# tensorflow/recommenders

Hardware: AMD Instinct MI355X
Metric: queries/sec brute-force top-100 (higher is better)
Workload: dtype f32; 1 GPU; BruteForce top-100, 1M-item x dim-64 corpus, batch 8192 (BASELINE.json configs[1]); corpus_rows_total=1000000, corpus_rows_per_gpu=1000000, dim=64, batch=8192, k=100, parallelism=single GPU

## Files before the change

recommenders_amd/csrc/topk_select16.hip:

```cpp
#include "common.h"

namespace tfrs {

constexpr int kSel16Waves = 4;
constexpr int kSlots = 16;
#ifndef TFRS_LIST16_ABLATE
#define TFRS_LIST16_ABLATE 0
#endif
#if TFRS_LIST16_ABLATE
#ifndef TFRS_ALLOW_ABLATION
#error "TFRS_LIST16_ABLATE != 0 is a measurement build with wrong results: add -DTFRS_ALLOW_ABLATION to confirm"
#endif
extern "C" int tfrs_ablation_build_list16(void) { return TFRS_LIST16_ABLATE; }
#endif
constexpr int kRadixBits = 24;

__device__ __forceinline__ uint32_t sel16_mbcnt(uint64_t mask) {
  return __builtin_amdgcn_mbcnt_hi((uint32_t)(mask >> 32),
                                   __builtin_amdgcn_mbcnt_lo((uint32_t)mask, 0u));
}
__device__ __forceinline__ void sel16_lds_sync() {
  __builtin_amdgcn_fence(__ATOMIC_ACQ_REL, "wavefront");
  __builtin_amdgcn_wave_barrier();
}

__device__ __forceinline__ uint32_t radix_kth(const uint32_t (&key)[kSlots], int k, int nslots = kSlots) {
  uint32_t kmax = 0u, kmin = 0xFFFFFFFFu;
  int n = 0;
#pragma unroll
  for (int s = 0; s < kSlots; ++s)
    if (s < nslots) {
      kmax = max(kmax, key[s]);
      kmin = min(kmin, key[s] != 0u ? key[s] : 0xFFFFFFFFu);
      n += (int)__popcll(__ballot(key[s] != 0u));
    }
  if (n < k) return 0u;
#pragma unroll
  for (int off = 32; off > 0; off >>= 1) {
    kmax = max(kmax, (uint32_t)__shfl_xor((int)kmax, off));
    kmin = min(kmin, (uint32_t)__shfl_xor((int)kmin, off));
  }
  kmax = __builtin_amdgcn_readfirstlane(kmax);
  kmin = __builtin_amdgcn_readfirstlane(kmin);
  constexpr uint32_t kLowBits = (1u << (32 - kRadixBits)) - 1u;
  const uint32_t diff = kmax ^ kmin;
  if ((diff & ~kLowBits) == 0u) return kmax & ~kLowBits;
  const int top = 31 - __builtin_clz(diff);
  uint32_t prefix = top == 31 ? 0u : (kmax & ~((2u << top) - 1u));
#pragma unroll 1
  for (int bit = top; bit >= 32 - kRadixBits; --bit) {
    const uint32_t test = prefix | (1u << bit);
    const uint32_t himask = ~((1u << bit) - 1u);
    int cnt = 0;
#pragma unroll
    for (int s = 0; s < kSlots; ++s)
      if (s < nslots) cnt += (int)__popcll(__ballot((key[s] & himask) == test));
    if (cnt >= k) prefix = test; else k -= cnt;
  }
  return prefix;
}

__global__ void __launch_bounds__(kSel16Waves * 64) bin_threshold_kernel(
    const float *__restrict__ binmax, int64_t ld, int n_bins, int group, int64_t nq, int k,
    const float *__restrict__ qk, const float *__restrict__ norm_max, float *__restrict__ lower,
    float *__restrict__ raw) {
  const int lane = threadIdx.x & 63;
  const int64_t row = (int64_t)blockIdx.x * kSel16Waves + (threadIdx.x >> 6);
  if (row >= nq) return;
  const float *src = binmax + row * ld;
  uint32_t key[kSlots];
  if (group == 1) {
    float v[kSlots];
#pragma unroll
    for (int s = 0; s < kSlots; ++s) {
      const int b = s * 64 + lane;
      v[s] = src[b < n_bins ? b : n_bins - 1];
    }
#pragma unroll
    for (int s = 0; s < kSlots; ++s) key[s] = (s * 64 + lane < n_bins) ? f32_orderable(v[s]) : 0u;
  } else
#pragma unroll
  for (int s = 0; s < kSlots; ++s) {
    const int b0 = (s * 64 + lane) * group;
    float m = -__builtin_inff();
    if (group % 4 == 0) {
      for (int g = 0; g < group; g += 4) {
        if (b0 + g + 3 < n_bins) {
          const float4 v = *reinterpret_cast<const float4 *>(src + b0 + g);
          m = fmaxf(fmaxf(m, fmaxf(v.x, v.y)), fmaxf(v.z, v.w));
        } else {
          for (int e = 0; e < 4; ++e)
            if (b0 + g + e < n_bins) m = fmaxf(m, src[b0 + g + e]);
        }
      }
    } else {
      for (int g = 0; g < group; ++g)
        if (b0 + g < n_bins) m = fmaxf(m, src[b0 + g]);
    }
    key[s] = (b0 < n_bins) ? f32_orderable(m) : 0u;
  }
  const int nslots = min(kSlots, (n_bins + group * 64 - 1) / (group * 64));
  const uint32_t kth = radix_kth(key, k, nslots);
  if (lane == 0) {
    const float eps = qk[row] * norm_max[0] + kF16Tiny;
    const bool have = kth > f32_orderable(-__builtin_inff());
    lower[row] = have ? f32_from_orderable(kth) - eps : -__builtin_inff();
    raw[row] = have ? f32_from_orderable(kth) : -__builtin_inff();
  }
}

int launch_bin_threshold(const float *binmax, int64_t ld, int n_bins, int64_t nq, int k,
                         const float *qk, const float *norm_max, float *lower, float *raw,
                         hipStream_t stream) {
  if (nq <= 0) return TFRS_OK;
  int group = 1;
  if (n_bins > 64 * kSlots) group = ((n_bins + 64 * kSlots - 1) / (64 * kSlots) + 3) / 4 * 4;
  hipLaunchKernelGGL(bin_threshold_kernel, dim3((unsigned)((nq + kSel16Waves - 1) / kSel16Waves)),
                     dim3(kSel16Waves * 64), 0, stream, binmax, ld, n_bins, group, nq, k, qk,
                     norm_max, lower, raw);
  TFRS_LAUNCH_CHECK();
  return TFRS_OK;
}

__device__ __forceinline__ float packed_score16(const char *packed, int64_t row, int dp,
                                                const float *qs) {
  const float4 *ev = reinterpret_cast<const float4 *>(packed + row * (int64_t)row_bytes(dp));
  const float4 *od = ev + dp / 8;
  const float4 *q4 = reinterpret_cast<const float4 *>(qs);
  float acc = 0.0f;
#pragma unroll 4
  for (int m = 0; m < dp / 8; ++m) {
    const float4 e = ev[m], o = od[m];
    const float4 qa = q4[2 * m], qb = q4[2 * m + 1];
    acc = __builtin_fmaf(e.x, qa.x, acc);
    acc = __builtin_fmaf(o.x, qa.y, acc);
    acc = __builtin_fmaf(e.y, qa.z, acc);
    acc = __builtin_fmaf(o.y, qa.w, acc);
    acc = __builtin_fmaf(e.z, qb.x, acc);
    acc = __builtin_fmaf(o.z, qb.y, acc);
    acc = __builtin_fmaf(e.w, qb.z, acc);
    acc = __builtin_fmaf(o.w, qb.w, acc);
  }
  return acc;
}

template <int P>
__device__ __forceinline__ void sort_desc16(uint64_t *x, int lane) {
#pragma unroll 1
  for (int size = 2; size <= P; size <<= 1) {
#pragma unroll 1
    for (int stride = size >> 1; stride > 0; stride >>= 1) {
      for (int t = lane; t < P / 2; t += 64) {
        const int i = 2 * t - (t & (stride - 1));
        const int jx = i + stride;
        const bool desc = ((i & size) == 0);
        const uint64_t va = x[i], vb = x[jx];
        if ((va < vb) == desc) {
          x[i] = vb;
          x[jx] = va;
        }
      }
      sel16_lds_sync();
    }
  }
}

struct List16Args {
  int64_t nq;
  int k;
  const float *q;
  int d;
  const char *packed;
  const uint2 *buf;
  const uint32_t *cnt;
  uint32_t cap_l;
  int nseg;
  const float *qk;
  const float *norm_max;
  float *out_scores;
  int32_t *out_idx;
  uint32_t *redo;
  int64_t idx_base;
  const uint32_t *ovf_cnt;
  const uint2 *ovf_buf;
  uint32_t ovf_cap;
  const int32_t *rowmap;
  const float *verify_raw;
  uint32_t *redo_reason;
  const RawTable *raw;
};

template <int KP>
__global__ void __launch_bounds__(kSel16Waves * 64) list_topk16_kernel(const List16Args a) {
  extern __shared__ __attribute__((aligned(16))) char smem[];
  const int lane = threadIdx.x & 63;
  const int wave = __builtin_amdgcn_readfirstlane(threadIdx.x >> 6);
  const int64_t row = (int64_t)blockIdx.x * kSel16Waves + wave;
  if (row >= a.nq) return;
  constexpr int kCap = 64 * kSlots;
  uint2 *ent = reinterpret_cast<uint2 *>(smem) + (size_t)wave * kCap;
  uint64_t *ex = reinterpret_cast<uint64_t *>(ent);
  float *qs = reinterpret_cast<float *>(smem + (size_t)kSel16Waves * kCap * sizeof(uint2)) +
              (size_t)wave * TFRS_MAX_DIM;
  const int K = a.k;
  const int dp = padded_dim(a.d);
  for (int i = lane; i < dp; i += 64) qs[i] = (i < a.d) ? a.q[row * a.d + i] : 0.0f;

  const uint2 *qbuf = a.buf + (row * (int64_t)a.cap_l) * a.nseg;
  int total = 0;
  bool bad = false;
  auto push = [&](bool p, uint2 v) __attribute__((always_inline)) {
    const uint64_t mask = __ballot(p);
    const int pos = total + (int)sel16_mbcnt(mask);
    if (p && pos < kCap) ent[pos] = v;
    total += (int)__popcll(mask);
  };
  constexpr int kCntBatch = 16;
  if (a.nseg <= 64) {
    const int lseg = lane < a.nseg ? lane : a.nseg - 1;
    const uint32_t ecap = a.cap_l - 1u;
    uint32_t c = a.cnt[row * a.nseg + lseg];
    if (lane >= a.nseg) c = 0u;
    if (a.ovf_cnt) {
      bad = c > a.cap_l + kOvfPerSeg;
      c = min(c, a.cap_l);
    } else {
      bad = c > a.cap_l;
    }
    if (__ballot(bad) == 0ull) {
      for (uint32_t e0 = 0; __ballot(e0 < c) != 0ull; e0 += 8) {
        uint2 w[8];
#pragma unroll
        for (int x = 0; x < 8; ++x) w[x] = qbuf[(int64_t)min(e0 + x, ecap) * a.nseg + lseg];
#pragma unroll
        for (int x = 0; x < 8; ++x) push(e0 + x < c, w[x]);
      }
    }
  } else
  for (int sb0 = 0; sb0 < a.nseg && !bad; sb0 += 64 * kCntBatch) {
    uint32_t cnts[kCntBatch];
#pragma unroll
    for (int b = 0; b < kCntBatch; ++b) {
      const int sg = sb0 + b * 64 + lane;
      cnts[b] = a.cnt[row * a.nseg + (sg < a.nseg ? sg : a.nseg - 1)];
    }
#pragma unroll
    for (int b = 0; b < kCntBatch; ++b)
      if (sb0 + b * 64 + lane >= a.nseg) cnts[b] = 0u;
#pragma unroll
    for (int b = 0; b < kCntBatch; ++b) {
      if (a.ovf_cnt) {
        bad = bad || (cnts[b] > a.cap_l + kOvfPerSeg);
        cnts[b] = min(cnts[b], a.cap_l);
      } else {
        bad = bad || (cnts[b] > a.cap_l);
      }
    }
    if (__ballot(bad) != 0ull) {
      bad = true;
      break;
    }
    uint2 v[kCntBatch][2];
#pragma unroll
    for (int b = 0; b < kCntBatch; ++b)
#pragma unroll
      for (int e = 0; e < 2; ++e) {
        const int sg = sb0 + b * 64 + lane;
        v[b][e] = qbuf[(int64_t)min((uint32_t)e, a.cap_l - 1u) * a.nseg + (sg < a.nseg ? sg : a.nseg - 1)];
      }
#pragma unroll
    for (int b = 0; b < kCntBatch; ++b) {
      if (sb0 + b * 64 >= a.nseg) break;
#pragma unroll
      for (int e = 0; e < 2; ++e) push((uint32_t)e < cnts[b], v[b][e]);
      for (uint32_t e0 = 2; __ballot(e0 < cnts[b]) != 0ull; e0 += 4) {
        uint2 w[4];
#pragma unroll
        for (int x = 0; x < 4; ++x) {
          const int sg = sb0 + b * 64 + lane;
          w[x] = qbuf[(int64_t)min(e0 + x, a.cap_l - 1u) * a.nseg + (sg < a.nseg ? sg : a.nseg - 1)];
        }
#pragma unroll
        for (int x = 0; x < 4; ++x) push(e0 + x < cnts[b], w[x]);
      }
    }
  }
  if (a.ovf_cnt && __ballot(bad) == 0ull) {
    const uint32_t novf = a.ovf_cnt[row];
    if (novf > a.ovf_cap) bad = true;
    else
      for (uint32_t e0 = 0; e0 < novf; e0 += 64) {
        const bool p = e0 + lane < novf;
        push(p, p ? a.ovf_buf[row * (int64_t)a.ovf_cap + e0 + lane] : make_uint2(0u, 0u));
      }
  }
  const bool any_bad = __ballot(bad) != 0ull;
  if (lane == 0 && a.redo_reason && total > 3 * kCap / 4 && !any_bad)
    atomicMax(&a.redo_reason[3], (uint32_t)total);
  if (any_bad || total > kCap) {
    if (lane == 0) a.redo[1 + atomicAdd(a.redo, 1u)] = (uint32_t)row;
    if (lane == 0 && a.redo_reason) atomicAdd(&a.redo_reason[0], 1u);
    return;
  }
  sel16_lds_sync();
  if (TFRS_LIST16_ABLATE & 4) { if (lane == 0) a.out_idx[row * K] = total; return; }

  uint32_t key[kSlots], rowid[kSlots];
#pragma unroll
  for (int s = 0; s < kSlots; ++s) {
    const int e = s * 64 + lane;
    key[s] = 0u;
    rowid[s] = 0u;
    if (e < total) {
      const uint2 v = ent[e];
      key[s] = f32_orderable(__uint_as_float(v.x));
      rowid[s] = v.y;
    }
  }
  const float eps = a.qk[row] * a.norm_max[0] + kF16Tiny;
  const uint32_t kth = radix_kth(key, K, (total + 63) / 64);
  if (a.verify_raw && (kth == 0u || kth < f32_orderable(a.verify_raw[row]))) {
    if (lane == 0) a.redo[1 + atomicAdd(a.redo, 1u)] = (uint32_t)row;
    if (lane == 0 && a.redo_reason) atomicAdd(&a.redo_reason[1], 1u);
    return;
  }
  uint32_t lo_key = 0u;
  if (kth != 0u && eps < __builtin_inff()) lo_key = f32_orderable(f32_from_orderable(kth) - 2.0f * eps);
  sel16_lds_sync();

  uint32_t *keep = reinterpret_cast<uint32_t *>(ent);
  int m = 0;
#pragma unroll
  for (int s = 0; s < kSlots; ++s) {
    const bool kp = key[s] != 0u && key[s] >= lo_key;
    const uint64_t mask = __ballot(kp);
    const int pos = m + (int)sel16_mbcnt(mask);
    if (kp && pos < kCap) keep[pos] = rowid[s];
    m += (int)__popcll(mask);
  }
  if (m > KP) {
    if (lane == 0 && a.redo_reason) atomicAdd(&a.redo_reason[2], 1u);
    sel16_lds_sync();
    uint32_t kall[kSlots];
#pragma unroll
    for (int u = 0; u < kSlots; ++u) kall[u] = (u * 64 + lane < m) ? keep[u * 64 + lane] : 0u;
    sel16_lds_sync();
#pragma unroll 1
    for (int u = 0; u < kSlots; ++u) {
      uint64_t kk = 0ull;
      if (u * 64 + lane < m)
        kk = make_key(a.raw ? raw_score(a.raw, (int64_t)kall[u], a.d, qs) : packed_score16(a.packed, (int64_t)kall[u], dp, qs),
                      (int32_t)((a.rowmap ? (int64_t)a.rowmap[kall[u]] : (int64_t)kall[u]) + a.idx_base));
      ex[u * 64 + lane] = kk;
    }
    sel16_lds_sync();
    sort_desc16<kCap>(ex, lane);
    for (int i = lane; i < K; i += 64) {
      const uint64_t kk = ex[i];
      a.out_scores[row * K + i] = kk ? key_score(kk) : -__builtin_inff();
      a.out_idx[row * K + i] = kk ? key_index(kk) : -1;
    }
    return;
  }
  sel16_lds_sync();
  uint32_t kid[KP / 64];
#pragma unroll
  for (int u = 0; u < KP / 64; ++u) kid[u] = (u * 64 + lane < m) ? keep[u * 64 + lane] : 0u;
  sel16_lds_sync();
#pragma unroll
  for (int u = 0; u < KP / 64; ++u) {
    if (u * 64 < m) {
      uint64_t kk = 0ull;
      if (u * 64 + lane < m)
        kk = make_key((TFRS_LIST16_ABLATE & 1) ? (float)kid[u] * 1e-9f :
                      a.raw ? raw_score(a.raw, (int64_t)kid[u], a.d, qs) : packed_score16(a.packed, (int64_t)kid[u], dp, qs),
                      (int32_t)((a.rowmap ? (int64_t)a.rowmap[kid[u]] : (int64_t)kid[u]) + a.idx_base));
      ex[u * 64 + lane] = kk;
    }
  }
  for (int i = m + lane; i < KP; i += 64) ex[i] = 0ull;
  sel16_lds_sync();
  if (!(TFRS_LIST16_ABLATE & 2)) {
    if (KP > 128 && m <= 128) sort_desc16<128>(ex, lane); else sort_desc16<KP>(ex, lane);
  }

  for (int i = lane; i < K; i += 64) {
    const uint64_t kk = ex[i];
    a.out_scores[row * K + i] = kk ? key_score(kk) : -__builtin_inff();
    a.out_idx[row * K + i] = kk ? key_index(kk) : -1;
  }
}

template <int KP>
static int launch_list16_kp(const List16Args &a, hipStream_t stream) {
  const size_t lds = (size_t)kSel16Waves * (64 * kSlots * sizeof(uint2) + TFRS_MAX_DIM * sizeof(float)) *
                     ((TFRS_LIST16_ABLATE & 16) ? 2 : 1);
  const dim3 grid((unsigned)((a.nq + kSel16Waves - 1) / kSel16Waves));
  hipLaunchKernelGGL((list_topk16_kernel<KP>), grid, dim3(kSel16Waves * 64), lds, stream, a);
  TFRS_LAUNCH_CHECK();
  return TFRS_OK;
}

int launch_list_topk16(const float *q, int64_t nq, int d, const char *packed, const uint2 *buf,
                       const uint32_t *cnt, uint32_t cap_l, int nseg, int k, const float *qk,
                       const float *norm_max, float *out_scores, int32_t *out_idx, uint32_t *redo,
                       int64_t idx_base, const uint32_t *ovf_cnt, const uint2 *ovf_buf,
                       uint32_t ovf_cap, const int32_t *rowmap, const float *verify_raw,
                       uint32_t *redo_reason, hipStream_t stream, const RawTable *raw) {
  if (nq <= 0) return TFRS_OK;
  List16Args a;
  a.raw = raw;
  a.idx_base = idx_base;
  a.nq = nq;
  a.k = k;
  a.q = q;
  a.d = d;
  a.packed = packed;
  a.buf = buf;
  a.cnt = cnt;
  a.cap_l = cap_l;
  a.nseg = nseg;
  a.qk = qk;
  a.norm_max = norm_max;
  a.out_scores = out_scores;
  a.out_idx = out_idx;
  a.redo = redo;
  a.ovf_cnt = ovf_cnt;
  a.ovf_buf = ovf_buf;
  a.ovf_cap = ovf_cap;
  a.rowmap = rowmap;
  a.verify_raw = verify_raw;
  a.redo_reason = redo_reason;
  const int need = 2 * k;
  if (need <= 128) return launch_list16_kp<128>(a, stream);
  if (need <= 256) return launch_list16_kp<256>(a, stream);
  if (need <= 512) return launch_list16_kp<512>(a, stream);
  return launch_list16_kp<1024>(a, stream);
}

}
```

Measured before the change: 7.997 million queries/s.

## Process two query rows per wave to overlap selection with rescoring

Adds a PAIR variant of the list top-k kernel where each wave handles two rows. For half the waves, the second row's candidate gather and selection runs before the first row's rescore and sort, so memory latency from one row's phase can hide behind another's compute. Query values are held in registers and written to LDS only when rescoring. A host-side occupancy query enables pairing only when the batch exceeds one resident wave of work. This adds register pressure and possible occupancy loss from keeping two rows of state live, and adds more kernel template instantiations.

```diff
diff --git a/recommenders_amd/csrc/topk_select16.hip b/recommenders_amd/csrc/topk_select16.hip
--- a/recommenders_amd/csrc/topk_select16.hip
+++ b/recommenders_amd/csrc/topk_select16.hip
@@ -1,4 +1,7 @@
 #include "common.h"
+
+#include <map>
+#include <mutex>
 
 namespace tfrs {
 
@@ -13,6 +16,7 @@
 #endif
 extern "C" int tfrs_ablation_build_list16(void) { return TFRS_LIST16_ABLATE; }
 #endif
+constexpr int kPairB = 2;
 constexpr int kRadixBits = 24;
 
 __device__ __forceinline__ uint32_t sel16_mbcnt(uint64_t mask) {
@@ -190,21 +194,33 @@
   const RawTable *raw;
 };
 
-template <int KP>
+template <int KP, bool PAIR>
 __global__ void __launch_bounds__(kSel16Waves * 64) list_topk16_kernel(const List16Args a) {
   extern __shared__ __attribute__((aligned(16))) char smem[];
   const int lane = threadIdx.x & 63;
   const int wave = __builtin_amdgcn_readfirstlane(threadIdx.x >> 6);
-  const int64_t row = (int64_t)blockIdx.x * kSel16Waves + wave;
-  if (row >= a.nq) return;
   constexpr int kCap = 64 * kSlots;
+  constexpr int kQr = TFRS_MAX_DIM / 64;
   uint2 *ent = reinterpret_cast<uint2 *>(smem) + (size_t)wave * kCap;
   uint64_t *ex = reinterpret_cast<uint64_t *>(ent);
   float *qs = reinterpret_cast<float *>(smem + (size_t)kSel16Waves * kCap * sizeof(uint2)) +
               (size_t)wave * TFRS_MAX_DIM;
   const int K = a.k;
   const int dp = padded_dim(a.d);
-  for (int i = lane; i < dp; i += 64) qs[i] = (i < a.d) ? a.q[row * a.d + i] : 0.0f;
+  auto put_q = [&](const float (&qreg)[kQr]) __attribute__((always_inline)) {
+#pragma unroll
+    for (int c = 0; c < kQr; ++c)
+      if (c * 64 + lane < dp) qs[c * 64 + lane] = qreg[c];
+    sel16_lds_sync();
+  };
+
+  auto select = [&](const int64_t row, uint32_t (&kid)[KP / 64], float (&qreg)[kQr]) __attribute__((always_inline)) -> int {
+#pragma unroll
+  for (int c = 0; c < kQr; ++c) qreg[c] = (c * 64 + lane < a.d) ? a.q[row * a.d + c * 64 + lane] : 0.0f;
+  const float qk_row = a.qk[row], nmax = a.norm_max[0];
+  const float raw_bound = a.verify_raw ? a.verify_raw[row] : 0.0f;
+  const uint32_t novf = a.ovf_cnt ? a.ovf_cnt[row] : 0u;
+  sel16_lds_sync();
 
   const uint2 *qbuf = a.buf + (row * (int64_t)a.cap_l) * a.nseg;
   int total = 0;
@@ -216,7 +232,7 @@
     total += (int)__popcll(mask);
   };
   constexpr int kCntBatch = 16;
-  if (a.nseg <= 64) {
+  if (PAIR || a.nseg <= 64) {
     const int lseg = lane < a.nseg ? lane : a.nseg - 1;
     const uint32_t ecap = a.cap_l - 1u;
     uint32_t c = a.cnt[row * a.nseg + lseg];
@@ -236,7 +252,7 @@
         for (int x = 0; x < 8; ++x) push(e0 + x < c, w[x]);
       }
     }
-  } else
+  } else if constexpr (!PAIR)
   for (int sb0 = 0; sb0 < a.nseg && !bad; sb0 += 64 * kCntBatch) {
     uint32_t cnts[kCntBatch];
 #pragma unroll
@@ -286,7 +302,6 @@
     }
   }
   if (a.ovf_cnt && __ballot(bad) == 0ull) {
-    const uint32_t novf = a.ovf_cnt[row];
     if (novf > a.ovf_cap) bad = true;
     else
       for (uint32_t e0 = 0; e0 < novf; e0 += 64) {
@@ -300,10 +315,10 @@
   if (any_bad || total > kCap) {
     if (lane == 0) a.redo[1 + atomicAdd(a.redo, 1u)] = (uint32_t)row;
     if (lane == 0 && a.redo_reason) atomicAdd(&a.redo_reason[0], 1u);
-    return;
+    return -1;
   }
   sel16_lds_sync();
-  if (TFRS_LIST16_ABLATE & 4) { if (lane == 0) a.out_idx[row * K] = total; return; }
+  if (TFRS_LIST16_ABLATE & 4) { if (lane == 0) a.out_idx[row * K] = total; return -1; }
 
   uint32_t key[kSlots], rowid[kSlots];
 #pragma unroll
@@ -317,12 +332,12 @@
       rowid[s] = v.y;
     }
   }
-  const float eps = a.qk[row] * a.norm_max[0] + kF16Tiny;
+  const float eps = qk_row * nmax + kF16Tiny;
   const uint32_t kth = radix_kth(key, K, (total + 63) / 64);
-  if (a.verify_raw && (kth == 0u || kth < f32_orderable(a.verify_raw[row]))) {
+  if (a.verify_raw && (kth == 0u || kth < f32_orderable(raw_bound))) {
     if (lane == 0) a.redo[1 + atomicAdd(a.redo, 1u)] = (uint32_t)row;
     if (lane == 0 && a.redo_reason) atomicAdd(&a.redo_reason[1], 1u);
-    return;
+    return -1;
   }
   uint32_t lo_key = 0u;
   if (kth != 0u && eps < __builtin_inff()) lo_key = f32_orderable(f32_from_orderable(kth) - 2.0f * eps);
@@ -340,7 +355,7 @@
   }
   if (m > KP) {
     if (lane == 0 && a.redo_reason) atomicAdd(&a.redo_reason[2], 1u);
-    sel16_lds_sync();
+    put_q(qreg);
     uint32_t kall[kSlots];
 #pragma unroll
     for (int u = 0; u < kSlots; ++u) kall[u] = (u * 64 + lane < m) ? keep[u * 64 + lane] : 0u;
@@ -360,13 +375,21 @@
       a.out_scores[row * K + i] = kk ? key_score(kk) : -__builtin_inff();
       a.out_idx[row * K + i] = kk ? key_index(kk) : -1;
     }
-    return;
+    return -1;
   }
   sel16_lds_sync();
-  uint32_t kid[KP / 64];
 #pragma unroll
   for (int u = 0; u < KP / 64; ++u) kid[u] = (u * 64 + lane < m) ? keep[u * 64 + lane] : 0u;
   sel16_lds_sync();
+  return m;
+  };
+
+  auto rescore = [&](const int64_t row, const uint32_t (&kid)[KP / 64], const int m, const float (&qreg)[kQr])
+                     __attribute__((always_inline)) {
+  uint32_t orig[KP / 64];
+#pragma unroll
+  for (int u = 0; u < KP / 64; ++u) orig[u] = (a.rowmap && u * 64 + lane < m) ? (uint32_t)a.rowmap[kid[u]] : kid[u];
+  put_q(qreg);
 #pragma unroll
   for (int u = 0; u < KP / 64; ++u) {
     if (u * 64 < m) {
@@ -374,7 +397,7 @@
       if (u * 64 + lane < m)
         kk = make_key((TFRS_LIST16_ABLATE & 1) ? (float)kid[u] * 1e-9f :
                       a.raw ? raw_score(a.raw, (int64_t)kid[u], a.d, qs) : packed_score16(a.packed, (int64_t)kid[u], dp, qs),
-                      (int32_t)((a.rowmap ? (int64_t)a.rowmap[kid[u]] : (int64_t)kid[u]) + a.idx_base));
+                      (int32_t)((int64_t)(int32_t)orig[u] + a.idx_base));
       ex[u * 64 + lane] = kk;
     }
   }
@@ -389,14 +412,67 @@
     a.out_scores[row * K + i] = kk ? key_score(kk) : -__builtin_inff();
     a.out_idx[row * K + i] = kk ? key_index(kk) : -1;
   }
+  };
+
+  uint32_t kid[KP / 64];
+  float qreg[kQr];
+  if constexpr (!PAIR) {
+    const int64_t row = (int64_t)blockIdx.x * kSel16Waves + wave;
+    if (row < a.nq) {
+      const int m = select(row, kid, qreg);
+      if (m >= 0) rescore(row, kid, m, qreg);
+    }
+  } else {
+    const bool wave_b = ((wave + (int)blockIdx.x) & (kSel16Waves - 1)) < kPairB;
+    uint32_t kid_p[KP / 64];
+    float qreg_p[kQr];
+    const int64_t row0 = (int64_t)blockIdx.x * 2 * kSel16Waves + wave, row1 = row0 + kSel16Waves;
+    int m0 = row0 < a.nq ? select(row0, kid_p, qreg_p) : -1;
+    if (!wave_b && m0 >= 0) {
+      rescore(row0, kid_p, m0, qreg_p);
+      m0 = -1;
+    }
+    const int m1 = row1 < a.nq ? select(row1, kid, qreg) : -1;
+    if (m0 >= 0) rescore(row0, kid_p, m0, qreg_p);
+    if (m1 >= 0) rescore(row1, kid, m1, qreg);
+  }
+}
+
+template <int KP, bool PAIR>
+static int64_t list16_resident_wgs(size_t lds) {
+  static std::mutex mu;
+  static std::map<int, int64_t> known;
+  int dev = 0;
+  if (hipGetDevice(&dev) != hipSuccess) return 0;
+  std::lock_guard<std::mutex> lock(mu);
+  auto it = known.find(dev);
+  if (it != known.end()) return it->second;
+  int per_cu = 0, cus = 0;
+  if (hipOccupancyMaxActiveBlocksPerMultiprocessor(&per_cu, reinterpret_cast<const void *>(&list_topk16_kernel<KP, PAIR>),
+                                                   kSel16Waves * 64, lds) != hipSuccess ||
+      hipDeviceGetAttribute(&cus, hipDeviceAttributeMultiprocessorCount, dev) != hipSuccess)
+    per_cu = cus = 0;
+  return known[dev] = (int64_t)per_cu * cus;
 }
 
 template <int KP>
 static int launch_list16_kp(const List16Args &a, hipStream_t stream) {
   const size_t lds = (size_t)kSel16Waves * (64 * kSlots * sizeof(uint2) + TFRS_MAX_DIM * sizeof(float)) *
                      ((TFRS_LIST16_ABLATE & 16) ? 2 : 1);
+  const char *opt = option("TFRS_LIST16_PAIR");
+  bool pair = KP <= 512 && a.nseg <= 64 && !(opt && opt[0] == '0');
+  if (pair && !(opt && opt[0] == '1')) {
+    const int64_t resident = list16_resident_wgs<KP, false>(lds);
+    pair = resident > 0 && a.nq > kSel16Waves * resident;
+  }
+  if constexpr (KP <= 512) if (pair) {
+    const dim3 grid((unsigned)((a.nq + 2 * kSel16Waves - 1) / (2 * kSel16Waves)));
+    hipLaunchKernelGGL((list_topk16_kernel<KP, true>), grid, dim3(kSel16Waves * 64), lds, stream, a);
+    TFRS_LAUNCH_CHECK();
+    return TFRS_OK;
+  }
   const dim3 grid((unsigned)((a.nq + kSel16Waves - 1) / kSel16Waves));
-  hipLaunchKernelGGL((list_topk16_kernel<KP>), grid, dim3(kSel16Waves * 64), lds, stream, a);
+  hipLaunchKernelGGL((list_topk16_kernel<KP, false>), grid, dim3(kSel16Waves * 64), lds, stream, a);
   TFRS_LAUNCH_CHECK();
   return TFRS_OK;
 }
```

Result: no change. 8.069 million queries/s, median of 6 (+0.9%).
